# xmindflow/cenet

Measured on AMD Instinct MI355X. Metric: training images/sec (224x224, 4-class), higher is better.
Workload: dtype bf16

## Files before the change

cenet_amd/csrc/attn_diff.hip:

```cpp
#include "common.h"
#include "../../include/cenet_hip.h"
#include <cstdlib>

typedef bf16_t bf;
#define DA_NEG (-1.0e30f)
#define DA_LOG2E 1.4426950408889634f

#ifdef CENET_HOSTSIM_BUILD
__device__ __forceinline__ float da_exp2(float x) { return exp2f(x); }
__device__ __forceinline__ bool da_any(bool v) {
  int x = v ? 1 : 0;
#pragma unroll
  for (int o = 32; o > 0; o >>= 1) x |= __shfl_xor(x, o);
  return x != 0;
}
#else
__device__ __forceinline__ float da_exp2(float x) { return __builtin_amdgcn_exp2f(x); }
__device__ __forceinline__ bool da_any(bool v) { return __any(v); }
typedef short da_s4 __attribute__((ext_vector_type(4)));
#endif
__device__ __forceinline__ float da_max3(float a, float b, float c3) { return fmaxf(fmaxf(a, b), c3); }
__device__ __forceinline__ void da_wave_sync() {
#ifdef CENET_HOSTSIM_BUILD
  hipsim::wave_barrier();
// ... 980 lines not shown
  const int q00 = (bid.x * 4 + wave) * 32 * a.tiles;
  for (int t = 0; t < a.tiles; ++t) {
    const int q0 = q00 + 32 * t;
    if (q0 >= Nq) break;
    const int qi = q0 + r < Nq ? q0 + r : Nq - 1;
    bf16x8 qf[4];
#pragma unroll
    for (int ks = 0; ks < 4; ++ks) qf[ks] = da_ld8(qb + (long)qi * C + 16 * ks + 8 * hh, true);
    f32x16 S[2];
#pragma unroll
    for (int kt = 0; kt < 2; ++kt) {
      S[kt] = da_zero();
      if (32 * kt < Nk) {
#pragma unroll
        for (int ks = 0; ks < 4; ++ks) S[kt] = DA_MFMA(da_rm(Kimg + 32 * kt * KP, KP, r, 16 * ks, hh), qf[ks], S[kt]);
      }
#pragma unroll
      for (int i = 0; i < 16; ++i)
        if (32 * kt + da_row(i, hh) >= Nk) S[kt][i] = DA_NEG;
    }
    float mx = DA_NEG;
#pragma unroll
    for (int kt = 0; kt < 2; ++kt)
#pragma unroll
      for (int i = 0; i < 16; ++i) mx = fmaxf(mx, S[kt][i]);
    mx = fmaxf(mx, __shfl_xor(mx, 32));
    const float mc = mx * c;
    float l = 0.f;
#pragma unroll
    for (int kt = 0; kt < 2; ++kt)
#pragma unroll
      for (int i = 0; i < 16; ++i) {
        const float pv = da_exp2(S[kt][i] * c - mc);
        S[kt][i] = pv;
        l += pv;
      }
    l += __shfl_xor(l, 32);
    f32x16 O[2] = {da_zero(), da_zero()};
#pragma unroll
    for (int kt = 0; kt < 2; ++kt) {
      if (32 * kt >= Nk) continue;
      const bf* Vt = Vimg + 32 * kt * KP;
#pragma unroll
      for (int s2 = 0; s2 < 2; ++s2) {
        const bf16x8 pB = da_pack8(S[kt], s2);
#pragma unroll
        for (int dt = 0; dt < 2; ++dt) O[dt] = DA_MFMA(da_tr(Vt, KP, s2, 32 * dt, lane), pB, O[dt]);
      }
    }
    if (q0 + r < Nq) {
      const float inv = 1.f / l;
      bf* op = ob + (long)qi * C;
#pragma unroll
      for (int dt = 0; dt < 2; ++dt)
#pragma unroll
        for (int g = 0; g < 4; ++g) {
          float o4[4];
#pragma unroll
          for (int i = 0; i < 4; ++i) o4[i] = O[dt][4 * g + i] * inv;
          st4v(op + 32 * dt + 8 * g + 4 * hh, o4);
        }
      if (hh == 0) a.lse[((long)b * a.H + h) * Nq + qi] = mx * a.scale + logf(l);
    }
  }
}

extern "C" int cenet_sra_attn_fwd_bf16(const bf* q, const bf* kv, bf* o, float* lse, int B, int H, int Nq, int Nk, float scale,
                                       hipStream_t stream) {
  if (!q || !kv || !o || !lse || B <= 0 || H <= 0 || Nq <= 0) return CENET_EINVAL;
  if (!(Nk >= 1 && Nk <= 64)) return CENET_EUNSUPPORTED;
  if ((((uintptr_t)q | (uintptr_t)kv | (uintptr_t)o) & 15) != 0) return CENET_EINVAL;
  SraFwdArgs a;
  a.q = q; a.kv = kv; a.o = o; a.lse = lse; a.B = B; a.H = H; a.Nq = Nq; a.Nk = Nk; a.C = 64 * H; a.scale = scale;
  static const char* e = getenv("CENET_SRA_FWD_TILES");
  int tiles = 1;
  while (tiles < 8 && (long)cdiv(Nq, 128 * tiles) * B * H > 1024) ++tiles;
  if (e) tiles = atoi(e);
  a.tiles = tiles < 1 ? 1 : tiles;
  CENET_LAUNCH(sra_fwd_kernel, dim3(cdiv(Nq, 128 * a.tiles), B * H), dim3(256), stream, a);
  CENET_CHECK_LAUNCH();
  return CENET_OK;
}

extern "C" int cenet_sra_attn_bwd_supported(int hd, int Nk) { return hd == 64 && Nk >= 1 && Nk <= 64; }
extern "C" int cenet_sra_attn_bwd_blocks_supported(int hd, int Nk) { return hd == 64 && Nk > 64 && Nk <= 256; }

static int sra_tiles(int B, int H, int Nq) {
  static const char* e = getenv("CENET_SRA_TILES");
  int tiles = 1;
  while (tiles < 8 && (long)cdiv(Nq, 128 * tiles) * B * H > 256) ++tiles;
  if (e) tiles = atoi(e);
  return tiles < 1 ? 1 : tiles;
}
extern "C" int cenet_sra_attn_bwd_direct_supported(int B, int H, int Nq, int Nk) {
  return cenet_sra_attn_bwd_supported(64, Nk) && B > 0 && H > 0 && Nq > 0 && cdiv(Nq, 128 * sra_tiles(B, H, Nq)) == 1;
}

static int sra_bwd_launch(const bf* q, const bf* kv, const bf* o, const bf* dout, const float* lse, bf* dq, float* dkv, bf* dkv_bf,
                          int B, int H, int Nq, int Nk, float scale, hipStream_t stream) {
  if (!q || !kv || !o || !dout || !lse || !dq || (!dkv && !dkv_bf) || B <= 0 || H <= 0 || Nq <= 0) return CENET_EINVAL;
  const bool blocks = cenet_sra_attn_bwd_blocks_supported(64, Nk);
  if (!cenet_sra_attn_bwd_supported(64, Nk) && !blocks) return CENET_EUNSUPPORTED;
  if ((((uintptr_t)q | (uintptr_t)kv | (uintptr_t)o | (uintptr_t)dout | (uintptr_t)dq) & 15) != 0) return CENET_EINVAL;
  SraArgs a;
  a.q = q; a.kv = kv; a.o = o; a.dout = dout; a.lse = lse; a.dq = dq; a.dkv = dkv; a.dkv_bf = dkv_bf;
  a.B = B; a.H = H; a.Nq = Nq; a.Nk = Nk; a.C = 64 * H; a.scale = scale;
  a.tiles = sra_tiles(B, H, Nq);
  if (blocks) {
    if (dkv_bf) return CENET_EUNSUPPORTED;
    int tq = 1;
    while (tq < 8 && (long)cdiv(Nq, 128 * tq) * B * H > 512) ++tq;
    a.tiles = tq;
    CENET_LAUNCH((sra_bwd_kernel<4, true, false>), dim3(cdiv(Nq, 128 * tq), B * H), dim3(256), stream, a);
    const int nkb = cdiv(Nk, 64);
    int tk = 1;
    while (tk < 16 && (long)cdiv(Nq, 128 * tk) * B * H * nkb > 256) ++tk;
    a.tiles = tk;
    CENET_LAUNCH((sra_bwd_kernel<1, false, true>), dim3(cdiv(Nq, 128 * tk), B * H, nkb), dim3(256), stream, a);
    CENET_CHECK_LAUNCH();
    return CENET_OK;
  }
  if (dkv_bf && cdiv(Nq, 128 * a.tiles) != 1) return CENET_EUNSUPPORTED;
  CENET_LAUNCH((sra_bwd_kernel<1, true, true>), dim3(cdiv(Nq, 128 * a.tiles), B * H), dim3(256), stream, a);
  CENET_CHECK_LAUNCH();
  return CENET_OK;
}

extern "C" int cenet_sra_attn_bwd_bf16(const bf* q, const bf* kv, const bf* o, const bf* dout, const float* lse, bf* dq, float* dkv,
                                       int B, int H, int Nq, int Nk, float scale, hipStream_t stream) {
  if (!dkv) return CENET_EINVAL;
  return sra_bwd_launch(q, kv, o, dout, lse, dq, dkv, nullptr, B, H, Nq, Nk, scale, stream);
}

extern "C" int cenet_sra_attn_bwd_direct_bf16(const bf* q, const bf* kv, const bf* o, const bf* dout, const float* lse, bf* dq,
                                              bf* dkv, int B, int H, int Nq, int Nk, float scale, hipStream_t stream) {
  if (!dkv) return CENET_EINVAL;
  return sra_bwd_launch(q, kv, o, dout, lse, dq, nullptr, dkv, B, H, Nq, Nk, scale, stream);
}
```

cenet_amd/kern.py:

```python
from __future__ import annotations

import ctypes as C
import math
from typing import Optional

import torch

from . import _lib
from ._lib import EpiT, MatT

ACT = {"none": 0, "relu": 1, "lrelu": 2, "gelu": 3, "silu": 4, "sigmoid": 5}


def _chk(*ts):
    for t in ts:
        if t is None:
            continue
        if isinstance(t, Ptr):
            t = t.t
        if t.dtype not in (torch.float32, torch.bfloat16, torch.int32, torch.int64, torch.uint8):
            raise TypeError(f"cenet_amd kernels take fp32 / bf16 tensors (int32 / int64 / uint8 for indices and masks); "
                            f"got {t.dtype}")
        if not t.is_cuda and not _lib.is_hostsim():
            raise RuntimeError("cenet_amd kernels run on the MI355X only: tensor is not on a CUDA/HIP device "
# ... 192 lines not shown
    return bool(_lib.lib().cenet_flash_attn_supported(int(D), int(Dv)))


def flashb_supported(D: int, Dv: int) -> bool:
    return D <= 64 and Dv <= 128


def flash_fwd(a: AttnT, bf16: bool = False):
    name = "cenet_flash_attn_fwd_bf16" if bf16 else "cenet_flash_attn_fwd_f32"
    _lib.check(getattr(_lib.lib(), name)(C.byref(a), stream()), name)


def flash_bwd(a: AttnT, bf16: bool = False):
    name = "cenet_flash_attn_bwd_bf16" if bf16 else "cenet_flash_attn_bwd_f32"
    _lib.check(getattr(_lib.lib(), name)(C.byref(a), stream()), name)


class DiffAttnT(C.Structure):
    _fields_ = [(n, C.c_void_p) for n in ("q", "k", "v", "U", "lse", "dU", "dq", "dk", "dv", "ws")] + \
               [(n, C.c_int) for n in ("B", "H", "N", "hd")] + [("scale", C.c_float), ("batch_mul", C.c_int)]


def diffattn_heads_supported(hd: int, N: int) -> bool:
    return bool(_lib.lib().cenet_diffattn_heads_supported(int(hd), int(N)))


def diffattn_heads_ws_bytes(B: int, H: int, N: int) -> int:
    fn = _lib.lib().cenet_diffattn_heads_ws_bytes
    fn.restype = C.c_long
    return int(fn(int(B), int(H), int(N)))


def diffattn_heads(a: DiffAttnT, backward: bool):
    name = "cenet_diffattn_heads_bwd_bf16" if backward else "cenet_diffattn_heads_fwd_bf16"
    _lib.check(getattr(_lib.lib(), name)(C.byref(a), stream()), name)


def attn64_ws_bytes(B: int, H: int, N: int) -> int:
    fn = _lib.lib().cenet_attn64_ws_bytes
    fn.restype = C.c_long
    return int(fn(int(B), int(H), int(N)))


def attn64(a: DiffAttnT, backward: bool):
    name = "cenet_attn64_bwd_bf16" if backward else "cenet_attn64_fwd_bf16"
    _lib.check(getattr(_lib.lib(), name)(C.byref(a), stream()), name)


def sra_attn_bwd_supported(hd: int, Nk: int) -> bool:
    return bool(_lib.lib().cenet_sra_attn_bwd_supported(int(hd), int(Nk)))


def sra_attn_bwd_blocks_supported(hd: int, Nk: int) -> bool:
    return bool(_lib.lib().cenet_sra_attn_bwd_blocks_supported(int(hd), int(Nk)))


def sra_attn_fwd(q, kv, o, lse, B, H, Nq, Nk, scale):
    _chk(q, kv, o, lse)
    assert q.dtype == BF16 and kv.dtype == BF16 and o.dtype == BF16 and lse.dtype == torch.float32
    rc = _lib.lib().cenet_sra_attn_fwd_bf16(P(q), P(kv), P(o), P(lse), B, H, Nq, Nk, C.c_float(scale), stream())
    _lib.check(rc, "cenet_sra_attn_fwd_bf16")


def sra_attn_bwd(q, kv, o, dout, lse, dq, dkv, B, H, Nq, Nk, scale):
    _chk(q, kv, o, dout, lse, dq, dkv)
    assert q.dtype == BF16 and kv.dtype == BF16 and dq.dtype == BF16 and dkv.dtype == torch.float32
    rc = _lib.lib().cenet_sra_attn_bwd_bf16(P(q), P(kv), P(o), P(dout), P(lse), P(dq), P(dkv), B, H, Nq, Nk, C.c_float(scale),
                                            stream())
    _lib.check(rc, "cenet_sra_attn_bwd_bf16")


def sra_attn_bwd_direct_supported(B, H, Nq, Nk) -> bool:
    return bool(_lib.lib().cenet_sra_attn_bwd_direct_supported(int(B), int(H), int(Nq), int(Nk)))


def sra_attn_bwd_direct(q, kv, o, dout, lse, dq, dkv, B, H, Nq, Nk, scale):
    _chk(q, kv, o, dout, lse, dq, dkv)
    assert q.dtype == BF16 and kv.dtype == BF16 and dq.dtype == BF16 and dkv.dtype == BF16
    rc = _lib.lib().cenet_sra_attn_bwd_direct_bf16(P(q), P(kv), P(o), P(dout), P(lse), P(dq), P(dkv), B, H, Nq, Nk,
                                                   C.c_float(scale), stream())
    _lib.check(rc, "cenet_sra_attn_bwd_direct_bf16")


def softmax_rows_fwd(x, y, rows, n):
    _chk(x, y)
    _call("cenet_softmax_rows_fwd_f32", x, y, L(rows), n)


def softmax_rows_bwd(y, dy, dx, rows, n):
    _chk(y, dy, dx)
    _call("cenet_softmax_rows_bwd_f32", y, dy, dx, L(rows), n)


def softmax_rows_finite_fwd(x, y, rows, n):
    _chk(x, y)
    _call("cenet_softmax_rows_finite_fwd_f32", x, y, L(rows), n)


def softmax_rows_finite_bwd(y, dy, x, dx, rows, n):
    _chk(y, dy, x, dx)
    _call("cenet_softmax_rows_finite_bwd_f32", y, dy, x, dx, L(rows), n)


def layernorm_fwd(x, gamma, beta, y, mean, rstd, rows, Cn, eps):
    _chk(x, gamma, beta, y, mean, rstd)
    _call("cenet_layernorm_fwd_f32", x, gamma, beta, y, mean, rstd, rows, Cn, float(eps))


def layernorm_bwd(dy, x, gamma, mean, rstd, dx, dgamma, dbeta, rows, Cn, dx_add=None):
    _chk(dy, x, gamma, mean, rstd, dx, dgamma, dbeta, dx_add)
    _call("cenet_layernorm_bwd_add_acc_f32", dy, x, gamma, mean, rstd, dx_add, dx, dgamma, dbeta, rows, Cn)


def layernorm_bwd_part_supported(dy, x, Cn) -> bool:
    return bool(is_bf16(dy) and is_bf16(x) and Cn % 8 == 0 and Cn <= 512 and dy.data_ptr() % 16 == 0 and x.data_ptr() % 16 == 0)


def layernorm_bwd_part(dy, x, gamma, mean, rstd, dx, rows, Cn, dx_add=None, bscale=None, dxs=None):
    _chk(dy, x, gamma, mean, rstd, dx, dx_add, bscale, dxs)
    nrows = int(_lib.lib().cenet_layernorm_bwd_part_rows(rows, Cn))
    part = torch.empty((nrows, 2 * Cn), device=dy.device, dtype=torch.float32)
    if bscale is None:
        _call("cenet_layernorm_bwd_add_part_bf16", dy, x, gamma, mean, rstd, dx_add, dx, part, rows, Cn)
    else:
        _call("cenet_layernorm_bwd_add_part_scaled_bf16", dy, x, gamma, mean, rstd, dx_add, dx, part, bscale,
              rows // bscale.numel(), dxs, rows, Cn)
    return part


def ln_fold_group(items):
    n = len(items)
    if n == 0:
        return
    parts = (C.c_void_p * n)(*[t[0].data_ptr() for t in items])
    dgs = (C.c_void_p * n)(*[t[1].data_ptr() for t in items])
    dbs = (C.c_void_p * n)(*[t[2].data_ptr() for t in items])
    nr = (C.c_int * n)(*[t[0].shape[0] for t in items])
    cs = (C.c_int * n)(*[t[0].shape[1] // 2 for t in items])
    rc = _lib.lib().cenet_ln_fold_group(parts, dgs, dbs, nr, cs, n, stream())
    _lib.check(rc, "cenet_ln_fold_group")


def bn_stats(x, sb, B, Cn, HW, ws, mean, var, rmean, rvar, momentum, nbt):
    _chk(x, ws, mean, var, rmean, rvar)
    _call("cenet_bn_stats_f32", x, L(sb), B, Cn, HW, ws, mean, var, rmean, rvar, float(momentum), nbt)


def bn1d_supported(B: int) -> bool:
    return bool(_lib.lib().cenet_bn1d_supported(int(B)))


def bn1d_train_fwd(z, zn, mean, var, rmean, rvar, momentum, nbt, eps, gamma, beta, B, Cn):
    _chk(z, zn, mean, var, rmean, rvar, gamma, beta)
    assert z.dtype == torch.float32 and zn.dtype == torch.float32
    _lib.check(_lib.lib().cenet_bn1d_train_fwd_f32(P(z), P(zn), P(mean), P(var), P(rmean), P(rvar), C.c_float(momentum), P(nbt),
                                                   C.c_float(eps), P(gamma), P(beta), int(B), int(Cn), stream()),
               "cenet_bn1d_train_fwd_f32")


def bn1d_bwd(dy, z, dz, mean, var, eps, gamma, dgamma, dbeta, B, Cn):
    _chk(dy, z, dz, mean, var, gamma, dgamma, dbeta)
    assert dy.dtype == torch.float32 and z.dtype == torch.float32
    _lib.check(_lib.lib().cenet_bn1d_bwd_acc_f32(P(dy), P(z), P(dz), P(mean), P(var), C.c_float(eps), P(gamma), P(dgamma), P(dbeta),
                                                 int(B), int(Cn), stream()), "cenet_bn1d_bwd_acc_f32")


# ... 822 lines not shown
```

cenet_amd/networks/cenet/pvtv2.py:

```python
from __future__ import annotations

import math
from functools import partial

import torch
import torch.nn as nn

from ... import ops


def _init_weights(m):
    if isinstance(m, nn.Linear):
        nn.init.trunc_normal_(m.weight, std=.02)
        if m.bias is not None:
            nn.init.zeros_(m.bias)
    elif isinstance(m, nn.LayerNorm):
        nn.init.ones_(m.weight)
        nn.init.zeros_(m.bias)
    elif isinstance(m, nn.Conv2d):
        fan_out = m.kernel_size[0] * m.kernel_size[1] * m.out_channels // m.groups
        nn.init.normal_(m.weight, 0.0, math.sqrt(2.0 / fan_out))
        if m.bias is not None:
            nn.init.zeros_(m.bias)


class DropPath(nn.Module):

    def __init__(self, drop_prob: float = 0.0):
        super().__init__()
        self.drop_prob = drop_prob

    def sample_scale(self, batch: int, device):
        if not self.training or self.drop_prob == 0.0:
            return None
        keep = 1.0 - self.drop_prob
        return torch.empty(batch, device=device, dtype=torch.float32).bernoulli_(keep).div_(keep)


class DWConv(nn.Module):

    def __init__(self, dim=768):
        super().__init__()
        self.dwconv = nn.Conv2d(dim, dim, 3, 1, 1, bias=True, groups=dim)


class Mlp(nn.Module):

    def __init__(self, in_features, hidden_features=None, out_features=None, act_layer=nn.GELU, drop=0.):
        super().__init__()
        out_features = out_features or in_features
        hidden_features = hidden_features or in_features
        self.fc1 = nn.Linear(in_features, hidden_features)
        self.dwconv = DWConv(hidden_features)
        self.fc2 = nn.Linear(hidden_features, out_features)
        self.apply(_init_weights)

    def forward(self, x, H, W, resid=None, bscale=None):
        h = ops.linear(x, self.fc1.weight, self.fc1.bias)
        h = ops.dwconv_tok(h, self.dwconv.dwconv.weight, self.dwconv.dwconv.bias, H, W, act="gelu")
        return ops.linear(h, self.fc2.weight, self.fc2.bias, resid=resid, bscale=bscale)


class Attention(nn.Module):

    def __init__(self, dim, num_heads=8, qkv_bias=False, qk_scale=None, attn_drop=0., proj_drop=0., sr_ratio=1):
        super().__init__()
        assert dim % num_heads == 0, f"dim {dim} should be divided by num_heads {num_heads}."
        self.dim, self.num_heads, self.sr_ratio = dim, num_heads, sr_ratio
        if qk_scale is not None:
            raise NotImplementedError("qk_scale override is not used by CENet")
        self.q = nn.Linear(dim, dim, bias=qkv_bias)
        self.kv = nn.Linear(dim, dim * 2, bias=qkv_bias)
        self.proj = nn.Linear(dim, dim)
        if sr_ratio > 1:
            self.sr = nn.Conv2d(dim, dim, kernel_size=sr_ratio, stride=sr_ratio)
            self.norm = nn.LayerNorm(dim)
        self.apply(_init_weights)

    def forward(self, x, H, W, resid=None, bscale=None):
        q, x = ops.linear(x, self.q.weight, self.q.bias, tap=True)
        if self.sr_ratio > 1:
            x_ = ops.sr_conv_ln(x, H, W, self.sr.weight, self.sr.bias, self.sr_ratio, self.norm.weight, self.norm.bias, self.norm.eps)
        else:
            x_ = x
        kv = ops.linear(x_, self.kv.weight, self.kv.bias)
        o = ops.sr_attention(q, kv, self.num_heads)
        return ops.linear(o, self.proj.weight, self.proj.bias, resid=resid, bscale=bscale)


class Block(nn.Module):

    def __init__(self, dim, num_heads, mlp_ratio=4., qkv_bias=False, qk_scale=None, drop=0., attn_drop=0.,
                 drop_path=0., act_layer=nn.GELU, norm_layer=nn.LayerNorm, sr_ratio=1):
        super().__init__()
        self.norm1 = norm_layer(dim)
        self.attn = Attention(dim, num_heads=num_heads, qkv_bias=qkv_bias, qk_scale=qk_scale, sr_ratio=sr_ratio)
        self.drop_path = DropPath(drop_path) if drop_path > 0. else nn.Identity()
        self.norm2 = norm_layer(dim)
        self.mlp = Mlp(in_features=dim, hidden_features=int(dim * mlp_ratio))
        self.apply(_init_weights)

    def _scale(self, x):
        pend = getattr(self, "_dp_pending", None)
        if pend:
            return pend.pop()
        if isinstance(self.drop_path, DropPath):
            return self.drop_path.sample_scale(x.shape[0], x.device)
        return None

    def forward(self, x, H, W):
        y, xr = ops.layernorm_res(x, self.norm1.weight, self.norm1.bias, self.norm1.eps)
        x = self.attn(y, H, W, resid=xr, bscale=self._scale(x))
        m = self.mlp
        if ops.pvt_mlp_supported(x, m.fc1.out_features, H, W):
            return ops.pvt_mlp(x, H, W, self.norm2.weight, self.norm2.bias, self.norm2.eps, m.fc1.weight, m.fc1.bias,
                               m.dwconv.dwconv.weight, m.dwconv.dwconv.bias, m.fc2.weight, m.fc2.bias, self._scale(x))
        y, xr = ops.layernorm_res(x, self.norm2.weight, self.norm2.bias, self.norm2.eps)
        x = self.mlp(y, H, W, resid=xr, bscale=self._scale(x))
        return x


class OverlapPatchEmbed(nn.Module):

    def __init__(self, img_size=224, patch_size=7, stride=4, in_chans=3, embed_dim=768):
        super().__init__()
        self.patch_size, self.stride = patch_size, stride
        self.in_chans = in_chans
        self.proj = nn.Conv2d(in_chans, embed_dim, kernel_size=patch_size, stride=stride, padding=patch_size // 2)
        self.norm = nn.LayerNorm(embed_dim)
        self.apply(_init_weights)

    def forward(self, x, tokens=None):
        H, W = x.shape[2:]
        k, s, p = self.patch_size, self.stride, self.patch_size // 2
        Ho, Wo = (H + 2 * p - k) // s + 1, (W + 2 * p - k) // s + 1
        if tokens is not None and k == 3 and tokens.dtype == torch.bfloat16:
            t = ops.conv2d_tok(tokens, H, W, self.proj.weight, self.proj.bias, stride=s, pad=p, out_layout="tok")
            t = ops.layernorm(t, self.norm.weight, self.norm.bias, self.norm.eps)
            return t, Ho, Wo
        expand = self.in_chans if (x.shape[1] == 1 and self.in_chans > 1) else 0
        if expand and x.dtype == torch.bfloat16:
            t = ops.conv2d_nchw(x, ops.chan_sum_weight(self.proj.weight), self.proj.bias, stride=s, pad=p, out_layout="tok")
        else:
            t = ops.conv2d_nchw(x, self.proj.weight, self.proj.bias, stride=s, pad=p, out_layout="tok", expand_channels=expand)
        t = ops.layernorm(t, self.norm.weight, self.norm.bias, self.norm.eps)
        return t, Ho, Wo


class PyramidVisionTransformerImpr(nn.Module):

    def __init__(self, img_size=224, patch_size=16, in_chans=3, num_classes=1000, embed_dims=[64, 128, 256, 512],
                 num_heads=[1, 2, 4, 8], mlp_ratios=[4, 4, 4, 4], qkv_bias=False, qk_scale=None, drop_rate=0.,
                 attn_drop_rate=0., drop_path_rate=0., norm_layer=nn.LayerNorm, depths=[3, 4, 6, 3],
                 sr_ratios=[8, 4, 2, 1]):
        super().__init__()
        self.depths = depths
        dpr = [v.item() for v in torch.linspace(0, drop_path_rate, sum(depths))]
        cur = 0
        for s in range(4):
            pe = OverlapPatchEmbed(img_size=img_size // (1 if s == 0 else 2 ** (s + 1)), patch_size=7 if s == 0 else 3,
                                   stride=4 if s == 0 else 2, in_chans=in_chans if s == 0 else embed_dims[s - 1],
                                   embed_dim=embed_dims[s])
            setattr(self, f"patch_embed{s + 1}", pe)
        for s in range(4):
            blocks = nn.ModuleList([
                Block(dim=embed_dims[s], num_heads=num_heads[s], mlp_ratio=mlp_ratios[s], qkv_bias=qkv_bias,
                      qk_scale=qk_scale, drop_path=dpr[cur + i], norm_layer=norm_layer, sr_ratio=sr_ratios[s])
                for i in range(depths[s])])
# ... 99 lines not shown
```

cenet_amd/ops/attention.py:

```python
from __future__ import annotations

import contextlib
import math
import os
from typing import Optional, Sequence

import torch
from torch.autograd import Function

from .. import kern
from .infra import *
from .linear import *
from .norm import *
from .depthwise import *


class _AttnDesc:

    def __init__(self, B, H, Nq, Nk, D, Dv, scale, vdiv, qs, ks, vs, os_, qoff=0, koff=0, voff=0):
        self.B, self.H, self.Nq, self.Nk, self.D, self.Dv, self.scale, self.vdiv = B, H, Nq, Nk, D, Dv, scale, vdiv
        self.qs, self.ks, self.vs, self.os = qs, ks, vs, os_
        self.qoff, self.koff, self.voff = qoff, koff, voff
        self.finite = False

# ... 212 lines not shown
            lse = _empty((B, 2 * H, N), q)
            a = kern.DiffAttnT()
            a.q, a.k, a.v, a.U, a.lse = q.data_ptr(), k.data_ptr(), v.data_ptr(), U.data_ptr(), lse.data_ptr()
            a.B, a.H, a.N, a.hd, a.scale = B, H, N, hd, hd ** -0.5
            kern.diffattn_heads(a, backward=False)
            ctx.save_for_backward(q, k, v, U, lse)
            ctx.H = H
            return U
        if kern.flashb_supported(hd, dv) if _bf(q) else kern.flash_supported(hd, dv):
            d = _AttnDesc(B, 2 * H, N, N, hd, dv, hd ** -0.5, 2, (N * E, hd, E, 1), (N * E, hd, E, 1), (N * E, dv, E, 1),
                          (2 * H * N * dv, N * dv, dv, 1))
            d.finite = not _bf(q)
            kind, saved = _attn_forward(d, q, k, v, U)
            ctx.descs = [d]
            saved_list = [saved]
        else:
            ctx.descs, saved_list = [], []
            for s in (0, 1):
                d = _AttnDesc(B, H, N, N, hd, dv, hd ** -0.5, 1, (N * E, 2 * hd, E, 1), (N * E, 2 * hd, E, 1),
                              (N * E, dv, E, 1), (2 * H * N * dv, 2 * N * dv, dv, 1), qoff=s * hd, koff=s * hd)
                d.finite = not _bf(q)
                Us = U
                kind, saved = _attn_forward(d, q, k, v, _OffsetView(Us, s * N * dv))
                ctx.descs.append(d)
                saved_list.append(saved)
        ctx.kind = kind
        ctx.save_for_backward(q, k, v, U, *saved_list)
        ctx.H = H
        return U

    @staticmethod
    def backward(ctx, g):
        q, k, v, U = ctx.saved_tensors[:4]
        saved_list = ctx.saved_tensors[4:]
        g = _c(g)
        B, N, E = q.shape
        hd = E // ctx.H // 2
        dv = 2 * hd
        if ctx.pairs:
            H = ctx.H
            lse = saved_list[0]
            dqkv = torch.empty((3,) + tuple(q.shape), device=q.device, dtype=q.dtype)
            dq, dk, dvv = dqkv[0], dqkv[1], dqkv[2]
            ws = torch.empty(kern.diffattn_heads_ws_bytes(B, H, N), device=q.device, dtype=torch.uint8)
            a = kern.DiffAttnT()
            a.q, a.k, a.v, a.U, a.lse, a.dU = q.data_ptr(), k.data_ptr(), v.data_ptr(), U.data_ptr(), lse.data_ptr(), g.data_ptr()
            a.dq, a.dk, a.dv, a.ws = dq.data_ptr(), dk.data_ptr(), dvv.data_ptr(), ws.data_ptr()
            a.B, a.H, a.N, a.hd, a.scale = B, H, N, hd, hd ** -0.5
            kern.diffattn_heads(a, backward=True)
            return dq, dk, dvv, None
        dq = torch.empty_like(q)
        if len(ctx.descs) == 1:
            dvv = _zeros(v.shape, v)
            dk = _empty(k.shape, k) if _bf(k) else torch.empty_like(k)
            _attn_backward(ctx.descs[0], ctx.kind, saved_list[0], q, k, v, U, g, dq, dk, dvv)
            dk, dvv = kern.cast(dk, k.dtype), kern.cast(dvv, v.dtype)
        else:
            dk = torch.empty_like(k)
            dvv = None
            for s, (d, saved) in enumerate(zip(ctx.descs, saved_list)):
                tmp = torch.empty_like(v)
                _attn_backward(d, ctx.kind, saved, q, k, v, _OffsetView(U, s * N * dv), _OffsetView(g, s * N * dv), dq, dk, tmp)
                if dvv is None:
                    dvv = tmp
                else:
                    kern.copy_batched(tmp, 0, dvv, 0, 1, tmp.numel(), accumulate=True)
        return dq, dk, dvv, None


class _OffsetView:

    def __init__(self, t: Tensor, off: int):
        self._t, self._off = t, off
        self.device, self.dtype, self.is_cuda = t.device, t.dtype, t.is_cuda

    def data_ptr(self):
        return self._t.data_ptr() + kern.esz(self._t) * self._off


def sr_attention(q, kv, heads):
    return SRAttentionFn.apply(q, kv, heads)


def nonlocal_attention(theta, phi, g):
    return NonlocalAttnFn.apply(theta, phi, g)


class NonlocalAttnJointFn(Function):

    @staticmethod
    def forward(ctx, tpg):
        tpg = _c(tpg)
        B, C3 = tpg.shape[:2]
        Cn = C3 // 3
        N = tpg.numel() // (B * C3)
        ctx.tok64 = _bf(tpg) and Cn in (64, 128) and N >= 256
        ctx.dims = (B, Cn, N, tuple(tpg.shape))
        oshape = (B, Cn) + tuple(tpg.shape[2:])
        if ctx.tok64:
            T = torch.empty((B, 3, N, Cn), device=tpg.device, dtype=tpg.dtype)
            kern.transpose(tpg, Cn * N, T, Cn * N, 3 * B, Cn, N)
            U = torch.empty((B, 1, N, Cn), device=tpg.device, dtype=tpg.dtype)
            lse = torch.empty((B, 1, N), device=tpg.device, dtype=torch.float32)
            a = kern.DiffAttnT()
            e = T.element_size()
            a.q, a.k, a.v = T.data_ptr(), T.data_ptr() + e * N * Cn, T.data_ptr() + 2 * e * N * Cn
            a.U, a.lse = U.data_ptr(), lse.data_ptr()
            a.B, a.H, a.N, a.hd, a.scale, a.batch_mul = B, 1, N, Cn, Cn ** -0.5, 3
            kern.attn64(a, backward=False)
            o = torch.empty(oshape, device=tpg.device, dtype=tpg.dtype)
            kern.transpose(U, N * Cn, o, Cn * N, B, N, Cn)
            ctx.save_for_backward(T, U, lse)
            return o
        st, so = (3 * Cn * N, 0, 1, N), (Cn * N, 0, 1, N)
        d = _AttnDesc(B, 1, N, N, Cn, Cn, Cn ** -0.5, 1, st, st, st, so, qoff=0, koff=Cn * N, voff=2 * Cn * N)
        o = torch.empty(oshape, device=tpg.device, dtype=tpg.dtype)
        kind, saved = _attn_forward(d, tpg, tpg, tpg, o)
        ctx.save_for_backward(tpg, o, saved)
        ctx.d, ctx.kind = d, kind
        return o

    @staticmethod
    def backward(ctx, g):
        g = _c(g)
        B, Cn, N, shape = ctx.dims
        dj = torch.empty(shape, device=g.device, dtype=g.dtype)
        if ctx.tok64:
            T, U, lse = ctx.saved_tensors
            gt = torch.empty_like(U)
            kern.transpose(g, Cn * N, gt, N * Cn, B, Cn, N)
            dT = torch.empty_like(T)
            ws = torch.empty(kern.attn64_ws_bytes(B, 1, N), device=g.device, dtype=torch.uint8)
            a = kern.DiffAttnT()
            e = T.element_size()
            a.q, a.k, a.v = T.data_ptr(), T.data_ptr() + e * N * Cn, T.data_ptr() + 2 * e * N * Cn
            a.U, a.lse, a.dU = U.data_ptr(), lse.data_ptr(), gt.data_ptr()
            a.dq, a.dk, a.dv = dT.data_ptr(), dT.data_ptr() + e * N * Cn, dT.data_ptr() + 2 * e * N * Cn
            a.ws = ws.data_ptr()
            a.B, a.H, a.N, a.hd, a.scale, a.batch_mul = B, 1, N, Cn, Cn ** -0.5, 3
            kern.attn64(a, backward=True)
            kern.transpose(dT, N * Cn, dj, Cn * N, 3 * B, N, Cn)
            return dj
        tpg, o, saved = ctx.saved_tensors
        _attn_backward(ctx.d, ctx.kind, saved, tpg, tpg, tpg, o, g, dj, dj, dj)
        return dj


def nonlocal_attention_joint(tpg):
    return NonlocalAttnJointFn.apply(tpg)


def diff_attention_heads(q, k, v, H):
    return DiffAttnHeadsFn.apply(q, k, v, H)


class DiffAttnCombineFn(Function):

    @staticmethod
    def forward(ctx, U, lq1, lk1, lq2, lk2, lambda_init):
        U = _c(U)
        B, H2, N, dv = U.shape
        H = H2 // 2
        lam = _empty((3,), U)
        kern.diffattn_lambda_fwd(lq1, lk1, lq2, lk2, lambda_init, lam, lq1.numel())
        out = _act((B, N, H * dv), U)
        kern.diffattn_combine_fwd(U, lam, out, B, H, N, dv, 1e-5, 1.0 - lambda_init)
# ... 26 lines not shown
```

include/cenet_hip.h:

```cpp
#ifndef CENET_HIP_H
#define CENET_HIP_H

#ifdef __cplusplus
extern "C" {
#endif

#ifndef CENET_HOSTSIM_BUILD
typedef struct ihipStream_t* cenet_stream_t;
#else
typedef void* cenet_stream_t;
#endif

typedef struct {
  const void* ptr;
  long sb, sb2, skb, sr, sc;
  long sk_outer;
  int kinner;
  int mode, kfast;
  int patch_is_row, transposed;
  int KH, KW, Pw, Hs, Ws, stride, pad, dil;
  long sci, sy, sx;
} cenet_mat_t;

typedef struct {
// ... 26 lines not shown
  float* C;
  float* asum;
  long lda, ldb, skbA, skbB;
  int M, N, K, nkb;
  int akf, bkf;
} cenet_wgrad_prob_t;
long cenet_wgrad_group_ws_floats(const cenet_wgrad_prob_t* p, int n);
int cenet_wgrad_group_bf16(const cenet_wgrad_prob_t* p, int n, float* ws, long ws_floats, cenet_stream_t stream);
int cenet_wgrad_group_plan(const cenet_wgrad_prob_t* p, int n, int* launch, int* bm, int* bn, int* ns);
int cenet_wgrad_group_phase_bf16(const cenet_wgrad_prob_t* p, int n, float* ws, long ws_floats, int phase, cenet_stream_t stream);

int cenet_conv_direct_supported(int Cin, int Cout, int k, int stride, int pad);
int cenet_conv_direct_bf16(const unsigned short* x, const float* w, unsigned short* y, int B, int Cin, int Cout, int H, int W,
                           int k, int dgrad, cenet_stream_t stream);
int cenet_conv_c1_supported(int Cin, int Cout, int k, int stride, int pad);
int cenet_pw_fewout_supported(int Cin, int Cout);
int cenet_pw_fewout_wgrad_supported(int Cin, int Cout);
int cenet_pw_fewout_fwd_bf16(const unsigned short* x, const unsigned short* W, const float* bias, unsigned short* y, int B, int Cin,
    int Cout, long HW, cenet_stream_t stream);
int cenet_pw_fewout_dgrad_bf16(const unsigned short* dy, const unsigned short* W, unsigned short* dx, int B, int Cin, int Cout,
    long HW, cenet_stream_t stream);
int cenet_pw_fewout_wgrad_bf16(const unsigned short* x, const unsigned short* dy, float* dW_acc, float* dbias_acc, int B, int Cin,
    int Cout, long HW, cenet_stream_t stream);
int cenet_pw_small_supported(int G);
int cenet_pw_small_bf16(const unsigned short* x, const unsigned short* W, unsigned short* y, int B, int groups, int G, long HW,
    int transpose, cenet_stream_t stream);
int cenet_conv_c1_fwd_bf16(const unsigned short* x, const float* w, unsigned short* y, int B, int Cout, int H, int W, int k,
    cenet_stream_t stream);
int cenet_conv_c1_wgrad_bf16(const unsigned short* x, const unsigned short* dy, float* dw_acc, int B, int Cout, int H, int W,
    int k, cenet_stream_t stream);
int cenet_conv_wgrad_direct_supported(int Cin, int Cout, int k, int stride, int pad);
long cenet_conv_wgrad_direct_ws_floats(int Cin, int Cout, int k);
int cenet_conv_wgrad_direct_bf16(const unsigned short* x, const unsigned short* dy, float* dw_acc, float* ws, int B, int Cin,
                                 int Cout, int H, int W, int k, cenet_stream_t stream);

typedef struct {
  const void *q, *k, *v;
  void* o;
  float* lse;
  const void* dout;
  void *dq, *dk, *dv;
  float* delta;
  long qsb, qsh, qsi, qsd, ksb, ksh, ksi, ksd, vsb, vsh, vsi, vsd, osb, osh, osi, osd;
  int B, H, Nq, Nk, D, Dv, v_head_div;
  float scale;
  int dkv_zeroed;
  int dkv_f32;
  int finite_scores;
} cenet_attn_t;
int cenet_flash_attn_supported(int D, int Dv);
int cenet_flash_attn_fwd_f32(const cenet_attn_t* p, cenet_stream_t stream);
int cenet_flash_attn_bwd_f32(const cenet_attn_t* p, cenet_stream_t stream);
int cenet_flash_attn_fwd_bf16(const cenet_attn_t* p, cenet_stream_t stream);
int cenet_flash_attn_bwd_bf16(const cenet_attn_t* p, cenet_stream_t stream);
typedef struct {
  const void *q, *k, *v;
  void* U;
  float* lse;
  const void* dU;
  void *dq, *dk, *dv;
  void* ws;
  int B, H, N, hd;
  float scale;
  int batch_mul;
} cenet_diffattn_t;
int cenet_diffattn_heads_supported(int hd, int N);
long cenet_diffattn_heads_ws_bytes(int B, int H, int N);
int cenet_diffattn_heads_fwd_bf16(const cenet_diffattn_t* p, cenet_stream_t stream);
int cenet_diffattn_heads_bwd_bf16(const cenet_diffattn_t* p, cenet_stream_t stream);
long cenet_attn64_ws_bytes(int B, int H, int N);
int cenet_attn64_fwd_bf16(const cenet_diffattn_t* p, cenet_stream_t stream);
int cenet_attn64_bwd_bf16(const cenet_diffattn_t* p, cenet_stream_t stream);
int cenet_sra_attn_bwd_supported(int hd, int Nk);
int cenet_sra_attn_bwd_blocks_supported(int hd, int Nk);
int cenet_sra_attn_fwd_bf16(const unsigned short* q, const unsigned short* kv, unsigned short* o, float* lse, int B, int H, int Nq,
    int Nk, float scale, cenet_stream_t stream);
int cenet_sra_attn_bwd_bf16(const unsigned short* q, const unsigned short* kv, const unsigned short* o,
    const unsigned short* dout, const float* lse, unsigned short* dq, float* dkv, int B, int H, int Nq, int Nk, float scale,
    cenet_stream_t stream);
int cenet_sra_attn_bwd_direct_supported(int B, int H, int Nq, int Nk);
int cenet_sra_attn_bwd_direct_bf16(const unsigned short* q, const unsigned short* kv, const unsigned short* o,
    const unsigned short* dout, const float* lse, unsigned short* dq, unsigned short* dkv, int B, int H, int Nq, int Nk,
    float scale, cenet_stream_t stream);
int cenet_softmax_rows_fwd_f32(const float* x, float* y, long rows, int n, cenet_stream_t stream);
int cenet_softmax_rows_bwd_f32(const float* y, const float* dy, float* dx, long rows, int n, cenet_stream_t stream);
int cenet_softmax_rows_fwd_bf16(const float* x, unsigned short* y, long rows, int n, cenet_stream_t stream);
int cenet_softmax_rows_bwd_bf16(const unsigned short* y, const float* dy, unsigned short* dx, long rows, int n,
                                cenet_stream_t stream);
int cenet_softmax_rows_finite_fwd_f32(const float* x, float* y, long rows, int n, cenet_stream_t stream);
int cenet_softmax_rows_finite_bwd_f32(const float* y, const float* dy, const float* x, float* dx, long rows, int n,
                                      cenet_stream_t stream);

int cenet_layernorm_fwd_f32(const float* x, const float* gamma, const float* beta, float* y, float* mean, float* rstd,
                            int rows, int C, float eps, cenet_stream_t stream);
int cenet_layernorm_bwd_acc_f32(const float* dy, const float* x, const float* gamma, const float* mean, const float* rstd,
                                float* dx, float* dgamma_acc, float* dbeta_acc, int rows, int C, cenet_stream_t stream);
int cenet_layernorm_bwd_add_acc_f32(const float* dy, const float* x, const float* gamma, const float* mean, const float* rstd,
                                    const float* dx_add, float* dx, float* dgamma_acc, float* dbeta_acc, int rows, int C,
                                    cenet_stream_t stream);
#define CENET_BN_WS_FLOATS(C) (2L * (C) * 256)
int cenet_bn_stats_f32(const float* x, long sb, int B, int C, int HW, float* ws, float* mean, float* var,
                       float* running_mean, float* running_var, float momentum, long* num_batches_tracked,
                       cenet_stream_t stream);
int cenet_bn_apply_f32(const float* x, long sxb, float* y, long syb, const float* mean, const float* var, float eps,
                       const float* gamma, const float* beta, int act, float slope, int B, int C, int HW,
                       cenet_stream_t stream);
int cenet_bn_train_fwd_f32(const float* x, long sxb, float* y, long syb, float* ws, float* mean, float* var,
    float* running_mean, float* running_var, float momentum, long* num_batches_tracked, float eps, const float* gamma,
    const float* beta, int act, float slope, int B, int C, int HW, int nbt_count, cenet_stream_t stream);
int cenet_bn_bwd_acc_f32(const float* dy, long sgb, const float* x, long sxb, float* dx, long sdb, const float* mean,
                         const float* var, float eps, const float* gamma, const float* beta, int act, float slope, int B,
                         int C, int HW, float* ws, float* dgamma_acc, float* dbeta_acc, cenet_stream_t stream);
int cenet_bn_bwd_add_acc_f32(const float* dy, long sgb, const float* x, long sxb, float* dx, long sdb, const float* dx_add,
                             long sab, const float* mean, const float* var, float eps, const float* gamma, const float* beta,
                             int act, float slope, int B, int C, int HW, float* ws, float* dgamma_acc, float* dbeta_acc,
                             cenet_stream_t stream);

int cenet_bn1d_supported(int B);
int cenet_bn1d_train_fwd_f32(const float* z, float* zn, float* mean, float* var, float* running_mean, float* running_var,
                             float momentum, long* num_batches_tracked, float eps, const float* gamma, const float* beta, int B,
                             int C, cenet_stream_t stream);
int cenet_bn1d_bwd_acc_f32(const float* dy, const float* z, float* dz, const float* mean, const float* var, float eps,
                           const float* gamma, float* dgamma_acc, float* dbeta_acc, int B, int C, cenet_stream_t stream);

int cenet_dwconv3x3_nchw_f32(const float* x, long sxb, const float* w, const float* bias, float* y, long syb, float* a,
                             long sab, int B, int C, int H, int W, int dil, int flip, int act, float slope,
                             cenet_stream_t stream);
int cenet_dwconv3x3_tok_f32(const float* x, const float* w, const float* bias, float* y, float* a, int B, int C, int H, int W,
                            int flip, int act, float slope, cenet_stream_t stream);
int cenet_dwconv3x3_wgrad_nchw_acc_f32(const float* x, long sxb, const float* dy, long sgb, float* dw_acc, float* dbias_acc,
                                       int B, int C, int H, int W, int dil, cenet_stream_t stream);
int cenet_dwconv3x3_wgrad_tok_acc_f32(const float* x, const float* dy, float* dw_acc, float* dbias_acc, int B, int C, int H,
                                      int W, cenet_stream_t stream);

int cenet_layernorm_bwd_part_rows(int rows, int C);
int cenet_layernorm_bwd_add_part_bf16(const unsigned short* dy, const unsigned short* x, const float* gamma, const float* mean,
                                      const float* rstd, const unsigned short* dx_add, unsigned short* dx, float* part, int rows,
                                      int C, cenet_stream_t stream);
int cenet_layernorm_bwd_add_part_scaled_bf16(const unsigned short* dy, const unsigned short* x, const float* gamma,
                                             const float* mean, const float* rstd, const unsigned short* dx_add,
                                             unsigned short* dx, float* part, const float* bscale, int rows_per_sample,
                                             unsigned short* dxs, int rows, int C, cenet_stream_t stream);
int cenet_ln_fold_group(const void* const* part, float* const* dgamma_acc, float* const* dbeta_acc, const int* nrows, const int* C,
                        int n, cenet_stream_t stream);

int cenet_pvt_mlp_supported(int C, int HD, int H, int W);
int cenet_pvt_mlp_fwd_bf16(const unsigned short* x, const float* ln_g, const float* ln_b, float eps, const unsigned short* w1,
                           const float* b1, const float* wd, const float* bd, const unsigned short* w2, const float* b2,
                           const float* bscale, unsigned short* y, unsigned short* xn_out, float* mean_out, float* rstd_out,
                           unsigned short* h_out, unsigned short* a_out, int B, int H, int W, int C, int HD, cenet_stream_t stream);

long cenet_pvt_mlp_bwd_ws_floats(int B, int H, int W, int C);
int cenet_pvt_mlp_bwd_bf16(const unsigned short* g, const float* bscale, const unsigned short* w1, const unsigned short* w2,
                           const float* wd, const float* bd, const unsigned short* h, const unsigned short* x, const float* ln_g,
                           const float* mean, const float* rstd, unsigned short* gu, unsigned short* dh, unsigned short* dx,
                           const float* up_scale, unsigned short* dxs, float* dwd_acc, float* dbd_acc, float* dln_g_acc,
                           float* dln_b_acc, float* db2_acc, float* ws, int B, int H, int W, int C, int HD, cenet_stream_t stream);

int cenet_res_tail_supported(int H, int W);
int cenet_res_tail_fwd_bf16(const unsigned short* x2, const unsigned short* x3, const float* mean2, const float* var2,
                            const float* gamma2, const float* beta2, float eps2, const float* mean3, const float* var3,
                            const float* gamma3, const float* beta3, float eps3, const float* w, float slope, unsigned short* out,
                            int B, int C, int H, int W, cenet_stream_t stream);
long cenet_res_tail_bwd_ws_floats(int C);
int cenet_res_tail_bwd_bf16(const unsigned short* g, const unsigned short* x2, const unsigned short* x3, const float* mean2,
                            const float* var2, const float* gamma2, const float* beta2, float eps2, const float* mean3,
// ... 423 lines not shown
```

Before: 1833.

## Fuse SRA q-projection, attention and output projection into one kernel

Adds a HIP kernel that computes the q linear, the small-Nk SRA attention (softmax with lse) and the output projection with bias, bscale and residual in one pass, holding Wq, Wp, K and V in LDS. It is used for C=64/128 stages with Nk<=64, and the backward reuses the existing linear and attention backward through shim contexts. The goal is to remove two GEMM launches and the global round trips for q and o in the forward. In exchange, each block reloads full weights and K/V into LDS, occupancy is limited by the large LDS footprint, and q and o are still written out for the backward.

Result: no change. 1842, median of 6 (+0.5%).

```diff
diff --git a/cenet_amd/csrc/attn_diff.hip b/cenet_amd/csrc/attn_diff.hip
--- a/cenet_amd/csrc/attn_diff.hip
+++ b/cenet_amd/csrc/attn_diff.hip
@@ -1086,6 +1086,206 @@
   return CENET_OK;
 }
 
+struct SraQpArgs {
+  const bf *xn, *kv, *wq, *wp, *R;
+  const float *bq, *bp, *bscale;
+  bf *q, *o, *y;
+  float* lse;
+  int B, Nq, Nk, tiles;
+  float scale;
+};
+
+__device__ __forceinline__ bf16x8 da_rm44(const bf* img, int pitch, int row, int col, int hh) {
+  unsigned u[4];
+  memcpy(u, img + row * pitch + col + 4 * hh, 8);
+  memcpy(u + 2, img + row * pitch + col + 8 + 4 * hh, 8);
+  bf16x8 f;
+  memcpy(&f, u, 16);
+  return f;
+}
+
+template <int C>
+__global__ __launch_bounds__(256, C == 64 ? 2 : 1) void sra_qproj_fwd_kernel(SraQpArgs a) {
+  constexpr int H = C / 64, NT = C / 32, KS = C / 16, WP = C + 8, CH = C / 8;
+  constexpr int WIMG = C * WP, KVIMG = 64 * WP;
+  __shared__ __attribute__((aligned(16))) bf lds[2 * WIMG + 2 * KVIMG];
+  __shared__ float bias[2 * C];
+  const int tid = threadIdx.x, lane = tid & 63, wave = tid >> 6, r = lane & 31, hh = lane >> 5;
+  const cenet_bid bid = cenet_xcd_block();
+  const int b = bid.y;
+  const int Nq = a.Nq, Nk = a.Nk;
+  const float c = a.scale * DA_LOG2E;
+  const bf* xb = a.xn + (long)b * Nq * C;
+  const bf* kvb = a.kv + (long)b * Nk * 2 * C;
+  bf* Wq = lds;
+  bf* Wp = lds + WIMG;
+  bf* Kimg = lds + 2 * WIMG;
+  bf* Vimg = Kimg + KVIMG;
+  for (int id = tid; id < 2 * C * CH; id += 256) {
+    const int which = id / (C * CH), rem = id - which * (C * CH), row = rem / CH, c8 = rem - row * CH;
+    unsigned v4[4];
+    memcpy(v4, (which ? a.wp : a.wq) + row * C + 8 * c8, 16);
+    memcpy((which ? Wp : Wq) + row * WP + 8 * c8, v4, 16);
+  }
+  for (int id = tid; id < 2 * 64 * CH; id += 256) {
+    const int which = id / (64 * CH), rem = id - which * (64 * CH), row = rem / CH, c8 = rem - row * CH;
+    unsigned v4[4] = {0u, 0u, 0u, 0u};
+    if (row < Nk) memcpy(v4, kvb + (long)row * 2 * C + which * C + 8 * c8, 16);
+    memcpy((which ? Vimg : Kimg) + row * WP + 8 * c8, v4, 16);
+  }
+  for (int i = tid; i < 2 * C; i += 256) bias[i] = i < C ? (a.bq ? a.bq[i] : 0.f) : (a.bp ? a.bp[i - C] : 0.f);
+  __syncthreads();
+  const float bs = a.bscale ? a.bscale[b] : 1.f;
+  const int q00 = (bid.x * 4 + wave) * 32 * a.tiles;
+  for (int t = 0; t < a.tiles; ++t) {
+    const int q0 = q00 + 32 * t;
+    if (q0 >= Nq) break;
+    const int qi = q0 + r < Nq ? q0 + r : Nq - 1;
+    const bool qok = q0 + r < Nq;
+    const long row = ((long)b * Nq + qi) * C;
+    bf16x8 xf[KS];
+#pragma unroll
+    for (int ks = 0; ks < KS; ++ks) xf[ks] = da_ld8(xb + (long)qi * C + 16 * ks + 8 * hh, true);
+    f32x16 Y[NT];
+#pragma unroll
+    for (int nt = 0; nt < NT; ++nt) Y[nt] = da_zero();
+#pragma unroll
+    for (int h = 0; h < H; ++h) {
+      f32x16 Q[2];
+#pragma unroll
+      for (int m = 0; m < 2; ++m) {
+        Q[m] = da_zero();
+#pragma unroll
+        for (int ks = 0; ks < KS; ++ks) Q[m] = DA_MFMA(da_rm(Wq + (64 * h + 32 * m) * WP, WP, r, 16 * ks, hh), xf[ks], Q[m]);
+#pragma unroll
+        for (int i = 0; i < 16; ++i) Q[m][i] += bias[64 * h + 32 * m + da_row(i, hh)];
+        if (qok) {
+#pragma unroll
+          for (int g = 0; g < 4; ++g) {
+            float o4[4];
+#pragma unroll
+            for (int i = 0; i < 4; ++i) o4[i] = Q[m][4 * g + i];
+            st4v(a.q + row + 64 * h + 32 * m + 8 * g + 4 * hh, o4);
+          }
+        }
+      }
+      f32x16 S[2];
+#pragma unroll
+      for (int kt = 0; kt < 2; ++kt) {
+        S[kt] = da_zero();
+        if (32 * kt < Nk) {
+#pragma unroll
+          for (int m = 0; m < 2; ++m)
+#pragma unroll
+            for (int s2 = 0; s2 < 2; ++s2)
+              S[kt] = DA_MFMA(da_rm44(Kimg + 32 * kt * WP, WP, r, 64 * h + 32 * m + 16 * s2, hh), da_pack8(Q[m], s2), S[kt]);
+        }
+#pragma unroll
+        for (int i = 0; i < 16; ++i)
+          if (32 * kt + da_row(i, hh) >= Nk) S[kt][i] = DA_NEG;
+      }
+      float mx = DA_NEG;
+#pragma unroll
+      for (int kt = 0; kt < 2; ++kt)
+#pragma unroll
+        for (int i = 0; i < 16; ++i) mx = fmaxf(mx, S[kt][i]);
+      mx = fmaxf(mx, __shfl_xor(mx, 32));
+      const float mc = mx * c;
+      float l = 0.f;
+#pragma unroll
+      for (int kt = 0; kt < 2; ++kt)
+#pragma unroll
+        for (int i = 0; i < 16; ++i) {
+          const float pv = da_exp2(S[kt][i] * c - mc);
+          S[kt][i] = pv;
+          l += pv;
+        }
+      l += __shfl_xor(l, 32);
+      f32x16 O[2] = {da_zero(), da_zero()};
+#pragma unroll
+      for (int kt = 0; kt < 2; ++kt) {
+        if (32 * kt >= Nk) continue;
+        const bf* Vt = Vimg + 32 * kt * WP;
+#pragma unroll
+        for (int s2 = 0; s2 < 2; ++s2) {
+          const bf16x8 pB = da_pack8(S[kt], s2);
+#pragma unroll
+          for (int dt = 0; dt < 2; ++dt) O[dt] = DA_MFMA(da_tr(Vt, WP, s2, 64 * h + 32 * dt, lane), pB, O[dt]);
+        }
+      }
+      const float inv = 1.f / l;
+#pragma unroll
+      for (int dt = 0; dt < 2; ++dt) {
+#pragma unroll
+        for (int i = 0; i < 16; ++i) O[dt][i] *= inv;
+        if (qok) {
+#pragma unroll
+          for (int g = 0; g < 4; ++g) {
+            float o4[4];
+#pragma unroll
+            for (int i = 0; i < 4; ++i) o4[i] = O[dt][4 * g + i];
+            st4v(a.o + row + 64 * h + 32 * dt + 8 * g + 4 * hh, o4);
+          }
+        }
+      }
+      if (qok && hh == 0) a.lse[((long)b * H + h) * Nq + qi] = mx * a.scale + logf(l);
+#pragma unroll
+      for (int nt = 0; nt < NT; ++nt)
+#pragma unroll
+        for (int dt = 0; dt < 2; ++dt)
+#pragma unroll
+          for (int s2 = 0; s2 < 2; ++s2)
+            Y[nt] = DA_MFMA(da_rm44(Wp + 32 * nt * WP, WP, r, 64 * h + 32 * dt + 16 * s2, hh), da_pack8(O[dt], s2), Y[nt]);
+    }
+    if (qok) {
+#pragma unroll
+      for (int nt = 0; nt < NT; ++nt)
+#pragma unroll
+        for (int g = 0; g < 4; ++g) {
+          const int col = 32 * nt + 8 * g + 4 * hh;
+          float v[4];
+#pragma unroll
+          for (int i = 0; i < 4; ++i) v[i] = (Y[nt][4 * g + i] + bias[C + col + i]) * bs;
+          if (a.R) {
+            float rr[4];
+            ld4v(rr, a.R + row + col);
+#pragma unroll
+            for (int i = 0; i < 4; ++i) v[i] += rr[i];
+          }
+          st4v(a.y + row + col, v);
+        }
+    }
+  }
+}
+
+extern "C" int cenet_sra_qproj_supported(int C, int H, int Nk) {
+  return (C == 64 || C == 128) && H * 64 == C && Nk >= 1 && Nk <= 64;
+}
+
+extern "C" int cenet_sra_qproj_fwd_bf16(const bf* xn, const bf* wq, const float* bq, const bf* kv, const bf* wp, const float* bp,
+                                        const float* bscale, const bf* R, bf* q, bf* o, float* lse, bf* y, int B, int Nq, int Nk,
+                                        int C, float scale, hipStream_t stream) {
+  if (!xn || !wq || !kv || !wp || !q || !o || !lse || !y || B <= 0 || Nq <= 0) return CENET_EINVAL;
+  if (!cenet_sra_qproj_supported(C, C / 64, Nk)) return CENET_EUNSUPPORTED;
+  if ((((uintptr_t)xn | (uintptr_t)wq | (uintptr_t)kv | (uintptr_t)wp | (uintptr_t)R | (uintptr_t)q | (uintptr_t)o | (uintptr_t)y) &
+       15) != 0)
+    return CENET_EINVAL;
+  SraQpArgs a;
+  a.xn = xn; a.kv = kv; a.wq = wq; a.wp = wp; a.R = R; a.bq = bq; a.bp = bp; a.bscale = bscale;
+  a.q = q; a.o = o; a.y = y; a.lse = lse; a.B = B; a.Nq = Nq; a.Nk = Nk; a.scale = scale;
+  static const char* e = getenv("CENET_SRA_QPROJ_TILES");
+  const int cap = C == 64 ? 512 : 256;
+  int tiles = 1;
+  while (tiles < 8 && (long)cdiv(Nq, 128 * tiles) * B > cap) ++tiles;
+  if (e) tiles = atoi(e);
+  a.tiles = tiles < 1 ? 1 : tiles;
+  const dim3 grid(cdiv(Nq, 128 * a.tiles), B);
+  if (C == 64) CENET_LAUNCH(sra_qproj_fwd_kernel<64>, grid, dim3(256), stream, a);
+  else CENET_LAUNCH(sra_qproj_fwd_kernel<128>, grid, dim3(256), stream, a);
+  CENET_CHECK_LAUNCH();
+  return CENET_OK;
+}
+
 extern "C" int cenet_sra_attn_bwd_supported(int hd, int Nk) { return hd == 64 && Nk >= 1 && Nk <= 64; }
 extern "C" int cenet_sra_attn_bwd_blocks_supported(int hd, int Nk) { return hd == 64 && Nk > 64 && Nk <= 256; }
 
diff --git a/cenet_amd/kern.py b/cenet_amd/kern.py
--- a/cenet_amd/kern.py
+++ b/cenet_amd/kern.py
@@ -298,6 +298,28 @@
     _lib.check(rc, "cenet_sra_attn_bwd_direct_bf16")
 
 
+_SRA_NO_FUSE = [__import__("os").environ.get("CENET_SRA_NO_FUSE") is not None]
+
+
+def set_sra_fuse(on: bool) -> bool:
+    old = not _SRA_NO_FUSE[0]
+    _SRA_NO_FUSE[0] = not on
+    return old
+
+
+def sra_qproj_supported(C_: int, H: int, Nk: int) -> bool:
+    return not _SRA_NO_FUSE[0] and bool(_lib.lib().cenet_sra_qproj_supported(int(C_), int(H), int(Nk)))
+
+
+def sra_qproj_fwd(xn, wq_, bq, kv, wp, bp, bscale, R, q, o, lse, y, B, Nq, Nk, C_, scale):
+    _chk(xn, wq_, bq, kv, wp, bp, bscale, R, q, o, lse, y)
+    assert all(t.dtype == BF16 for t in (xn, wq_, kv, wp, q, o, y)) and (R is None or R.dtype == BF16)
+    assert all(t is None or t.dtype == torch.float32 for t in (bq, bp, bscale, lse))
+    rc = _lib.lib().cenet_sra_qproj_fwd_bf16(P(xn), P(wq_), P(bq), P(kv), P(wp), P(bp), P(bscale), P(R), P(q), P(o), P(lse), P(y),
+                                             B, Nq, Nk, C_, C.c_float(scale), stream())
+    _lib.check(rc, "cenet_sra_qproj_fwd_bf16")
+
+
 def softmax_rows_fwd(x, y, rows, n):
     _chk(x, y)
     _call("cenet_softmax_rows_fwd_f32", x, y, L(rows), n)
diff --git a/cenet_amd/networks/cenet/pvtv2.py b/cenet_amd/networks/cenet/pvtv2.py
--- a/cenet_amd/networks/cenet/pvtv2.py
+++ b/cenet_amd/networks/cenet/pvtv2.py
@@ -78,12 +78,19 @@
         self.apply(_init_weights)
 
     def forward(self, x, H, W, resid=None, bscale=None):
-        q, x = ops.linear(x, self.q.weight, self.q.bias, tap=True)
+        fused = ops.sra_qproj_supported(x, self.num_heads, (H // self.sr_ratio) * (W // self.sr_ratio))
+        if fused:
+            q, x = ops.sra_qproj_tap(x, self.q.weight, self.q.bias)
+        else:
+            q, x = ops.linear(x, self.q.weight, self.q.bias, tap=True)
         if self.sr_ratio > 1:
             x_ = ops.sr_conv_ln(x, H, W, self.sr.weight, self.sr.bias, self.sr_ratio, self.norm.weight, self.norm.bias, self.norm.eps)
         else:
             x_ = x
         kv = ops.linear(x_, self.kv.weight, self.kv.bias)
+        if fused:
+            return ops.sra_qproj(q, kv, self.q.weight, self.q.bias, self.proj.weight, self.proj.bias, self.num_heads,
+                                 resid=resid, bscale=bscale)
         o = ops.sr_attention(q, kv, self.num_heads)
         return ops.linear(o, self.proj.weight, self.proj.bias, resid=resid, bscale=bscale)
 
diff --git a/cenet_amd/ops/attention.py b/cenet_amd/ops/attention.py
--- a/cenet_amd/ops/attention.py
+++ b/cenet_amd/ops/attention.py
@@ -318,6 +318,69 @@
     return SRAttentionFn.apply(q, kv, heads)
 
 
+class SRAQTapFn(Function):
+
+    @staticmethod
+    def forward(ctx, x, W, b):
+        x = _c(x)
+        ctx.save_for_backward(x, W, None)
+        ctx.refs = (W, b)
+        ctx.has_resid = False
+        return x.view_as(x), x.view_as(x)
+
+    @staticmethod
+    def backward(ctx, dq, g_tap=None):
+        return LinearFn.backward(ctx, dq, g_tap)[:3]
+
+
+class _Ctx:
+
+    def __init__(self, saved, **kw):
+        self.saved_tensors = saved
+        self.__dict__.update(kw)
+
+
+class SRAQProjFn(Function):
+
+    @staticmethod
+    def forward(ctx, xq, kv, Wq, bq, Wp, bp, resid, bscale, heads):
+        xq, kv, resid = _c(xq), _c(kv), _c(resid)
+        B, N, Cn = xq.shape
+        Nk = kv.shape[1]
+        hd = Cn // heads
+        q, o, y = torch.empty_like(xq), torch.empty_like(xq), torch.empty_like(xq)
+        lse = _empty((B, heads, N), xq)
+        kern.sra_qproj_fwd(xq, kern.wq(Wq, xq), bq, kv, kern.wq(Wp, xq), bp, bscale, resid, q, o, lse, y, B, N, Nk, Cn, hd ** -0.5)
+        ctx.save_for_backward(q, kv, o, lse, Wp, bscale)
+        ctx.refs = (Wp, bp)
+        ctx.has_resid = resid is not None
+        ctx.d = _AttnDesc(B, heads, N, Nk, hd, hd, hd ** -0.5, 1, (N * Cn, hd, Cn, 1), (Nk * 2 * Cn, hd, 2 * Cn, 1),
+                          (Nk * 2 * Cn, hd, 2 * Cn, 1), (N * Cn, hd, Cn, 1), voff=Cn)
+        return y
+
+    @staticmethod
+    def backward(ctx, g):
+        q, kv, o, lse, Wp, bscale = ctx.saved_tensors
+        r = LinearFn.backward(_Ctx((o, Wp, bscale), refs=ctx.refs, has_resid=ctx.has_resid, needs_input_grad=(True,)), g)
+        dq, dkv, _ = SRAttentionFn.backward(_Ctx((q, kv, o, lse), d=ctx.d, kind="flash"), r[0])
+        return dq, dkv, None, None, None, None, r[3], None, None
+
+
+def sra_qproj_supported(x, heads, Nk):
+    return bool(x.dim() == 3 and _bf(x) and kern.sra_qproj_supported(x.shape[-1], heads, Nk))
+
+
+def sra_qproj_tap(x, Wq, bq):
+    return SRAQTapFn.apply(x, Wq, bq)
+
+
+def sra_qproj(xq, kv, Wq, bq, Wp, bp, heads, resid=None, bscale=None):
+    y = SRAQProjFn.apply(xq, kv, Wq, bq, Wp, bp, resid, bscale, heads)
+    if bscale is not None and resid is not None:
+        tag_bscale(y, bscale)
+    return y
+
+
 def nonlocal_attention(theta, phi, g):
     return NonlocalAttnFn.apply(theta, phi, g)
 
diff --git a/include/cenet_hip.h b/include/cenet_hip.h
--- a/include/cenet_hip.h
+++ b/include/cenet_hip.h
@@ -132,6 +132,10 @@
 int cenet_sra_attn_bwd_direct_bf16(const unsigned short* q, const unsigned short* kv, const unsigned short* o,
     const unsigned short* dout, const float* lse, unsigned short* dq, unsigned short* dkv, int B, int H, int Nq, int Nk,
     float scale, cenet_stream_t stream);
+int cenet_sra_qproj_supported(int C, int H, int Nk);
+int cenet_sra_qproj_fwd_bf16(const unsigned short* xn, const unsigned short* wq, const float* bq, const unsigned short* kv,
+    const unsigned short* wp, const float* bp, const float* bscale, const unsigned short* R, unsigned short* q,
+    unsigned short* o, float* lse, unsigned short* y, int B, int Nq, int Nk, int C, float scale, cenet_stream_t stream);
 int cenet_softmax_rows_fwd_f32(const float* x, float* y, long rows, int n, cenet_stream_t stream);
 int cenet_softmax_rows_bwd_f32(const float* y, const float* dy, float* dx, long rows, int n, cenet_stream_t stream);
 int cenet_softmax_rows_fwd_bf16(const float* x, unsigned short* y, long rows, int n, cenet_stream_t stream);
```
